# jeffreyhorn/network_flow_solver

Measured on AMD Instinct MI355X. Metric: pivots/sec + arcs-priced/sec (value = arcs-priced/sec; pivots_per_sec alongside) on netgen_8-style DIMACS, higher is better.
Workload: dtype int64; 1 GPU; netgen_8_08a(synthetic,x1): 256 nodes / 2048 arcs; pricing=full-scan Dantzig, step=one pivot (price + ratio test + tree/potential update), parallelism=1 GPU, sweeps=full (every arc priced every pivot)

## Files before the change

__graft_entry__.py:

```python

from __future__ import annotations

import os
import re
import subprocess
import sys
from pathlib import Path

ROOT = Path(__file__).resolve().parent
PKG = ROOT / "network_flow_solver_amd"
CSRC = PKG / "csrc"
LIB = PKG / "libmcf_hip.so"
CERT_HOST_LIB = PKG / "libmcf_certify_host.so"
REPAIR_HOST_LIB = PKG / "libmcf_repair_host.so"
FARKAS_HOST_LIB = PKG / "libmcf_farkas_host.so"
TOPOLOGY_HOST_LIB = PKG / "libmcf_topology_host.so"
RANGES_HOST_LIB = PKG / "libmcf_ranges_host.so"
FLOW_RANGES_HOST_LIB = PKG / "libmcf_flow_ranges_host.so"
DUAL_HOST_LIB = PKG / "libmcf_dual_host.so"
APPLY_PATHS_HOST_LIB = PKG / "libmcf_apply_paths_host.so"
SMALL_REDUCE_HOST_LIB = PKG / "libmcf_small_reduce_host.so"
SMALL_CYCLE_REGS_HOST_LIB = PKG / "libmcf_small_cycle_regs_host.so"
FORK_HOST_LIB = PKG / "libmcf_fork_host.so"
DECIDE_FLAT_HOST_LIB = PKG / "libmcf_decide_flat_host.so"
SMALL_SLOTS_HOST_LIB = PKG / "libmcf_small_slots_host.so"
SMALL_BUDGET_HOST_LIB = PKG / "libmcf_small_budget_host.so"

if str(ROOT) not in sys.path:
    sys.path.insert(0, str(ROOT))


def _hipcc() -> str:
    for cand in (os.environ.get("HIPCC"), "/opt/rocm/bin/hipcc", "hipcc"):
        if cand and (os.path.isabs(cand) and os.path.exists(cand) or not os.path.isabs(cand)):
            return cand
    return "hipcc"


def _needs_rebuild(target: Path, sources) -> bool:
    if not target.exists():
        return True
    t = target.stat().st_mtime
    return any(Path(s).stat().st_mtime > t for s in sources)


def build_hip(force: bool = False) -> Path:
    sources = [CSRC / "mcf_engine.hip", CSRC / "mcf_passes_dev.h", CSRC / "mcf_passes_host.h", CSRC / "mcf_core.h", CSRC / "mcf_host.h",
               ROOT / "include" / "mcf.h"]
    if force or _needs_rebuild(LIB, sources):
        cmd = [_hipcc(), "--offload-arch=gfx950", "-O3", "-std=c++17", "-fPIC", "-shared",
               "-o", str(LIB), str(CSRC / "mcf_engine.hip")]
        subprocess.run(cmd, check=True, cwd=str(CSRC))
    return LIB


def build_certify_host(force: bool = False) -> Path:
    src = CSRC / "mcf_certify_host.cpp"
    if force or _needs_rebuild(CERT_HOST_LIB, [src, CSRC / "mcf_core.h"]):
        subprocess.run(["g++", "-O2", "-std=c++17", "-fPIC", "-shared", "-o", str(CERT_HOST_LIB), str(src)], check=True, cwd=str(CSRC))
    return CERT_HOST_LIB


def build_repair_host(force: bool = False) -> Path:
    src = CSRC / "mcf_repair_host.cpp"
    if force or _needs_rebuild(REPAIR_HOST_LIB, [src, CSRC / "mcf_core.h", CSRC / "mcf_host.h"]):
        subprocess.run(["g++", "-O2", "-std=c++17", "-fPIC", "-shared", "-o", str(REPAIR_HOST_LIB), str(src)], check=True, cwd=str(CSRC))
    return REPAIR_HOST_LIB


def build_farkas_host(force: bool = False) -> Path:
    src = CSRC / "mcf_farkas_host.cpp"
    if force or _needs_rebuild(FARKAS_HOST_LIB, [src, CSRC / "mcf_core.h"]):
        subprocess.run(["g++", "-O2", "-std=c++17", "-fPIC", "-shared", "-o", str(FARKAS_HOST_LIB), str(src)], check=True, cwd=str(CSRC))
    return FARKAS_HOST_LIB


def build_topology_host(force: bool = False) -> Path:
    src = CSRC / "mcf_topology_host.cpp"
    if force or _needs_rebuild(TOPOLOGY_HOST_LIB, [src, CSRC / "mcf_core.h", CSRC / "mcf_host.h"]):
# ... 19 lines not shown
    src = CSRC / "mcf_dual_host.cpp"
    if force or _needs_rebuild(DUAL_HOST_LIB, [src, CSRC / "mcf_core.h", CSRC / "mcf_host.h", ROOT / "include" / "mcf.h"]):
        subprocess.run(["g++", "-O2", "-std=c++17", "-fPIC", "-shared", "-o", str(DUAL_HOST_LIB), str(src)], check=True, cwd=str(CSRC))
    return DUAL_HOST_LIB


def build_apply_paths_host(force: bool = False) -> Path:
    src = CSRC / "mcf_apply_paths_host.cpp"
    if force or _needs_rebuild(APPLY_PATHS_HOST_LIB, [src, CSRC / "mcf_core.h", CSRC / "mcf_host.h"]):
        subprocess.run(["g++", "-O2", "-std=c++17", "-fPIC", "-shared", "-o", str(APPLY_PATHS_HOST_LIB), str(src)], check=True, cwd=str(CSRC))
    return APPLY_PATHS_HOST_LIB


def build_small_reduce_host(force: bool = False) -> Path:
    src = CSRC / "mcf_small_reduce_host.cpp"
    if force or _needs_rebuild(SMALL_REDUCE_HOST_LIB, [src, CSRC / "mcf_core.h"]):
        subprocess.run(["g++", "-O2", "-std=c++17", "-fPIC", "-shared", "-o", str(SMALL_REDUCE_HOST_LIB), str(src)], check=True, cwd=str(CSRC))
    return SMALL_REDUCE_HOST_LIB


def build_small_cycle_regs_host(force: bool = False) -> Path:
    src = CSRC / "mcf_small_cycle_regs_host.cpp"
    if force or _needs_rebuild(SMALL_CYCLE_REGS_HOST_LIB, [src, CSRC / "mcf_core.h"]):
        subprocess.run(["g++", "-O2", "-std=c++17", "-fPIC", "-shared", "-o", str(SMALL_CYCLE_REGS_HOST_LIB), str(src)], check=True, cwd=str(CSRC))
    return SMALL_CYCLE_REGS_HOST_LIB


def build_fork_host(force: bool = False) -> Path:
    src = CSRC / "mcf_fork_host.cpp"
    if force or _needs_rebuild(FORK_HOST_LIB, [src, CSRC / "mcf_core.h"]):
        subprocess.run(["g++", "-O2", "-std=c++17", "-fPIC", "-shared", "-o", str(FORK_HOST_LIB), str(src)], check=True, cwd=str(CSRC))
    return FORK_HOST_LIB


def build_decide_flat_host(force: bool = False) -> Path:
    src = CSRC / "mcf_decide_flat_host.cpp"
    if force or _needs_rebuild(DECIDE_FLAT_HOST_LIB, [src, CSRC / "mcf_core.h"]):
        subprocess.run(["g++", "-O2", "-std=c++17", "-fPIC", "-shared", "-o", str(DECIDE_FLAT_HOST_LIB), str(src)], check=True, cwd=str(CSRC))
    return DECIDE_FLAT_HOST_LIB


def build_small_slots_host(force: bool = False) -> Path:
    src = CSRC / "mcf_small_slots_host.cpp"
    if force or _needs_rebuild(SMALL_SLOTS_HOST_LIB, [src, CSRC / "mcf_core.h"]):
        subprocess.run(["g++", "-O2", "-std=c++17", "-fPIC", "-shared", "-o", str(SMALL_SLOTS_HOST_LIB), str(src)], check=True, cwd=str(CSRC))
    return SMALL_SLOTS_HOST_LIB


def build_small_budget_host(force: bool = False) -> Path:
    src = CSRC / "mcf_small_budget_host.cpp"
    if force or _needs_rebuild(SMALL_BUDGET_HOST_LIB, [src, CSRC / "mcf_core.h", CSRC / "mcf_host.h"]):
        subprocess.run(["g++", "-O2", "-std=c++17", "-fPIC", "-shared", "-o", str(SMALL_BUDGET_HOST_LIB), str(src)], check=True, cwd=str(CSRC))
    return SMALL_BUDGET_HOST_LIB


def declared_symbols() -> list[str]:
    text = (ROOT / "include" / "mcf.h").read_text()
    text = re.sub(r"/\*.*?\*/", "", text, flags=re.S)
    names = re.findall(r"\b(mcf_[a-z0-9_]+)\s*\(", text)
    return sorted(set(n for n in names if n != "mcf_progress_cb"))


def build() -> None:
    build_hip()
    import oracle

    oracle.build()
    oracle.build_emul()
    build_certify_host()
    build_repair_host()
    build_farkas_host()
    build_topology_host()
    build_ranges_host()
    build_flow_ranges_host()
    build_dual_host()
    build_apply_paths_host()
    build_small_reduce_host()
    build_small_cycle_regs_host()
    build_fork_host()
    build_decide_flat_host()
    build_small_slots_host()
    build_small_budget_host()
    import ctypes

    lib = ctypes.CDLL(str(LIB))
    missing = [s for s in declared_symbols() if not hasattr(lib, s)]
    if missing:
        raise RuntimeError(f"libmcf_hip.so lacks symbols declared in include/mcf.h: {missing}")
    import network_flow_solver_amd


def smoke() -> None:
    import numpy as np

    build_hip()
    import oracle
    from network_flow_solver_amd import engine, generators

    if engine.device_count() <= 0:
        raise RuntimeError("smoke() needs a GPU: no HIP device visible")
    inst = generators.netgen_style(256, 2048, seed=7)
    ref = oracle.solve_soa(inst, "dantzig")
    for rule in (engine.RULE_DANTZIG, engine.RULE_DEVEX_BLOCK, engine.RULE_CANDIDATE_LIST):
        with engine.McfEngine(inst.n, inst.tail, inst.head, inst.cost, inst.cap, inst.supply, rule=rule,
                              device=0) as eng:
            eng.solve()
            res = eng.result()
        assert res.status == ref["status"] == "optimal", (res.status, ref["status"])
        assert res.objective == int(round(ref["objective"])), (res.objective, ref["objective"])
        bal = inst.supply.astype(np.int64).copy()
        np.subtract.at(bal, inst.tail, res.flow)
        np.add.at(bal, inst.head, res.flow)
        assert not bal.any()
        rc = inst.cost + res.potential[inst.tail] - res.potential[inst.head]
        assert (rc[(res.flow > 0) & (res.flow < inst.cap)] == 0).all()
        assert (rc[(res.flow == 0) & (inst.cap > 0)] >= 0).all() and (rc[(res.flow == inst.cap) & (inst.cap > 0)] <= 0).all()
        print(f"smoke ok: rule={rule} objective={res.objective} pivots={res.stats['pivots']} "
              f"(oracle {ref['iterations']} pivots)")


if __name__ == "__main__":
    build()
    if len(sys.argv) > 1 and sys.argv[1] == "smoke":
        smoke()
```

network_flow_solver_amd/csrc/mcf_core.h:

```cpp
#pragma once
#include <stdint.h>

#if defined(__HIPCC__)
#define MCF_HD __host__ __device__ __forceinline__
#else
#define MCF_HD inline
#endif

#define MCF_INF ((int64_t)1 << 60)

#if defined(__HIP_DEVICE_COMPILE__)
#define mcf_double_bits(x) ((int64_t)__double_as_longlong(x))
#else
static inline int64_t mcf_double_bits(double x) { int64_t k; __builtin_memcpy(&k, &x, 8); return k; }
#endif

#if defined(__HIP_DEVICE_COMPILE__)
#define MCF_TEAM_BARRIER() __syncthreads()
#define MCF_ATOMIC_MIN64(p, x) atomicMin(reinterpret_cast<long long*>(p), (long long)(x))
#define MCF_ATOMIC_MIN32(p, x) atomicMin(reinterpret_cast<int*>(p), (int)(x))
#define MCF_ATOMIC_MAX32(p, x) atomicMax(reinterpret_cast<int*>(p), (int)(x))
#define MCF_ATOMIC_ADD32(p, x) atomicAdd(reinterpret_cast<int*>(p), (int)(x))
#define MCF_ATOMIC_MAX64(p, x) atomicMax(reinterpret_cast<long long*>(p), (long long)(x))
#define MCF_ATOMIC_OR32(p, x) atomicOr(reinterpret_cast<int*>(p), (int)(x))
// ... 1917 lines not shown
    }
}

MCF_HD void mcf_apply_catch_up_store_at(int32_t* dst, int32_t* pnext, int32_t j, int32_t nd) {
    dst[j] = nd;
    pnext[nd] = j;
}
MCF_HD void mcf_apply_catch_up_store(const McfView& v, const McfCtx& c, int32_t j, int32_t nd) {
    (c.cur ? v.order[0] : v.order[1])[j] = nd;
    (c.cur ? v.posbuf[0] : v.posbuf[1])[nd] = j;
}

MCF_HD void mcf_apply_one_paths_at(const McfView& v, const McfCtx& c, const McfNode* srec, const int32_t* spos, const int32_t* src,
                                   int32_t* dst, int32_t* pnext, int32_t j) {
    if (j >= c.lo && j < c.hi) {
        bool in_t2;
        int32_t dd;
        const int32_t i = mcf_apply_source_paths(c, srec, spos, j, &in_t2, &dd);
        const int32_t nd = src[i];
        dst[j] = nd;
        pnext[nd] = j;
        if (in_t2) {
            const int64_t pot = v.pi[nd];
            const int32_t dep = v.node[nd].depth;
            v.pi[nd] = pot + c.sigma;
            if (dd) v.node[nd].depth = dep + dd;
        }
    } else {
        mcf_apply_catch_up_store_at(dst, pnext, j, src[j]);
    }
}
MCF_HD void mcf_apply_one_paths(const McfView& v, const McfCtx& c, const McfNode* srec, const int32_t* spos, int32_t j) {
    const int32_t* src = c.cur ? v.order[1] : v.order[0];
    int32_t* dst = c.cur ? v.order[0] : v.order[1];
    int32_t* pnext = c.cur ? v.posbuf[0] : v.posbuf[1];
    if (j >= c.lo && j < c.hi) {
        bool in_t2;
        int32_t dd;
        const int32_t i = mcf_apply_source_paths(c, srec, spos, j, &in_t2, &dd);
        const int32_t nd = src[i];
        dst[j] = nd;
        pnext[nd] = j;
        if (in_t2) {
            const int64_t pot = v.pi[nd];
            const int32_t dep = v.node[nd].depth;
            v.pi[nd] = pot + c.sigma;
            if (dd) v.node[nd].depth = dep + dd;
        }
    } else {
        mcf_apply_catch_up_store(v, c, j, src[j]);
    }
}

MCF_HD void mcf_reach_reindex_block(const McfView& v, const int32_t* zs, int32_t b) {
    int32_t m = 0;
    for (int32_t j = b << MCF_REACH_SHIFT; j < ((b + 1) << MCF_REACH_SHIFT) && j < v.n_nodes; ++j) {
        const int32_t e = j + zs[j];
        if (e > m) m = e;
    }
    v.reach[b] = m;
}

typedef unsigned __int128 mcf_u128;

#define MCF_CERT_BOUNDS 1u
#define MCF_CERT_CONSERVATION 2u
#define MCF_CERT_DUAL 4u
#define MCF_CERT_OBJECTIVES 8u
#define MCF_CERT_BASIS 16u
#define MCF_CERT_PRICING 32u
#define MCF_CERT_ALL 63u
#define MCF_CERT_NONE INT64_MAX

struct McfCertArcAcc {
    int64_t neg_n, over_n, bnd_w, bnd_i;
    int64_t dlo_n, dlo_w, dlo_i;
    int64_t dup_n, dup_w, dup_i;
    int64_t basic_n, stf_n;
    int64_t rc_n, rc_bad, key_n, key_bad;
    int64_t sat_n;
    uint64_t primal_lo, primal_hi;
    uint64_t dcap_lo, dcap_hi;
};
struct McfCertNodeAcc {
    int64_t imb_n, imb_w, imb_i;
    int64_t art_basic, tree_rc_bad, shape_bad, strong_bad;
    uint64_t art_lo, art_hi;
    uint64_t dnode_lo, dnode_hi;
};
template <typename Acc>
constexpr int mcf_acc_words() {
    static_assert(sizeof(Acc) % 8 == 0, "accumulators are whole 8-byte words");
    return (int)(sizeof(Acc) / 8);
}

MCF_HD void mcf_cert_arc_init(McfCertArcAcc* a) {
    uint64_t* p = reinterpret_cast<uint64_t*>(a);
    for (int k = 0; k < mcf_acc_words<McfCertArcAcc>(); ++k) p[k] = 0;
    a->bnd_i = a->dlo_i = a->dup_i = MCF_CERT_NONE;
}
MCF_HD void mcf_cert_node_init(McfCertNodeAcc* a) {
    uint64_t* p = reinterpret_cast<uint64_t*>(a);
    for (int k = 0; k < mcf_acc_words<McfCertNodeAcc>(); ++k) p[k] = 0;
    a->imb_i = MCF_CERT_NONE;
}
MCF_HD void mcf_cert_worst(int64_t* w, int64_t* wi, int64_t mag, int64_t idx) {
// ... 338 lines not shown
```

network_flow_solver_amd/csrc/mcf_engine.hip:

```cpp
#include <hip/hip_runtime.h>

#include <algorithm>
#include <cerrno>
#include <cstddef>
#include <chrono>
#include <cstdio>
#include <cstdlib>
#include <cstring>
#include <mutex>
#include <new>
#include <string>
#include <vector>

#include "../../include/mcf.h"
#include "mcf_core.h"
#include "mcf_host.h"

namespace {

constexpr int kPriceThreads = 256;
constexpr int kPivotThreads = 1024;
constexpr int kReduceThreads = 256;
constexpr int kMidMaxNodes = 1536;
constexpr int kMidMaxArcsPerPivot = MCF_TUNER_MAX_ARCS + 1024;
// ... 1358 lines not shown
#define MCF_WAVE_T0() do {} while (0)
#define MCF_WAVE_STAMP(slot) do {} while (0)
#define MCF_WAVE_PROBE(word) do {} while (0)
#endif

struct alignas(8) SmallCycleAcc {
    int32_t c[16][2];
};
constexpr bool small_search_join(int threads) { return threads != 256; }

template <bool LAST>
__device__ __forceinline__ void small_ratio_side(const int64_t* res, int32_t n, int64_t* d_out, int32_t* k_out) {
    const int32_t lane = (int32_t)(threadIdx.x & 63);
    int64_t d = MCF_INF;
    int32_t k = -1;
    const int64_t r0 = lane < n ? res[lane] : MCF_INF;
    bool wide = !mcf_ratio_narrow_ok(r0);
    for (int32_t i = 64 + lane; i < n; i += 64) wide |= !mcf_ratio_narrow_ok(res[i]);
    if (__ballot(wide) == 0) {
        for (int32_t base = 0; base < n; base += 64) {
            const int32_t i = base + lane;
            const uint32_t key = mcf_ratio_key32(base == 0 ? r0 : (i < n ? res[i] : MCF_INF));
            const uint32_t mn = mcf_wave_min_u32(key);
            const uint64_t mask = __ballot(i < n && key == mn);
            mcf_ratio_take<LAST>(mcf_ratio_unkey32(mn), mask, base, d, k);
        }
        *d_out = d; *k_out = k;
        return;
    }
    for (int32_t base = 0; base < n; base += 64) {
        const int32_t i = base + lane;
        const int64_t r = i < n ? res[i] : INT64_MAX;
        const int64_t mn = -mcf_wave_max64(-r);
        const uint64_t mask = __ballot(r == mn);
        mcf_ratio_take<LAST>(mn, mask, base, d, k);
    }
    *d_out = d; *k_out = k;
}

constexpr bool small_search_one_branch(int threads) { return threads == 256; }

constexpr bool small_ratio_together(int threads) { return threads == 256 || threads == 1024; }
constexpr bool small_record_once(int threads) { return threads == 256; }
typedef int small_i32x4 __attribute__((ext_vector_type(4)));
constexpr bool small_ratio_one_trip(int threads) { return threads == 256; }
typedef int small_i32x2 __attribute__((ext_vector_type(2)));
#ifndef MCF_BUDGET_OFF
#define MCF_BUDGET_OFF 0
#endif
constexpr bool small_pair_arith(int threads, bool front) { return threads == 256 && front && !(MCF_BUDGET_OFF & 1); }
constexpr bool small_ballot_direct(int threads, bool front) { return threads == 256 && front && !(MCF_BUDGET_OFF & 2); }
constexpr bool small_counts_packed(int threads, bool front) { return threads == 256 && front && !(MCF_BUDGET_OFF & 4); }
constexpr bool small_finish_one_trip(int threads, bool front) { return small_pair_arith(threads, front) && !(MCF_BUDGET_OFF & 8); }

template <int THREADS, bool FRONT>
__device__ __forceinline__ void small_cycle_parallel(const McfView& v, SmallCycleAcc& A, int64_t* scratch, McfCycle& cy) {
    constexpr bool kScalar = small_scalar_control(THREADS);
    constexpr bool kSearchJoin = small_search_join(THREADS);
    constexpr bool kSearchOneBranch = small_search_one_branch(THREADS);
    constexpr bool kRatioTogether = small_ratio_together(THREADS);
    constexpr bool kRecordOnce = small_record_once(THREADS);
    constexpr bool kRatioOneTrip = kRatioTogether && small_ratio_one_trip(THREADS);
    constexpr bool kPairs = small_pair_arith(THREADS, FRONT) && kSearchOneBranch;
    constexpr bool kBallot = small_ballot_direct(THREADS, FRONT) && kSearchOneBranch && !kSearchJoin && kRatioOneTrip;
    constexpr bool kCounts = small_counts_packed(THREADS, FRONT) && kRatioOneTrip;
    const McfCtx* c = v.ctx;
    const int32_t d4 = mcf_pair_dist4(v.n_nodes), d16 = mcf_pair_dist16(v.n_nodes);
    const int32_t* pcur = kPairs ? v.posbuf[0] + mcf_pair_index(0, c->cur, d4) : (c->cur ? v.posbuf[1] : v.posbuf[0]);
    const int32_t du0 = cy.r0u.depth, dw0 = cy.r0w.depth;
    const int32_t pu = cy.p0u, pw = cy.p0w;
    const int32_t wave = (int32_t)threadIdx.x >> 6;
    const int32_t N = v.n_nodes;
    int64_t* const res1 = scratch;
    int64_t* const res2 = res1 + N;
    int32_t* const by_depth = reinterpret_cast<int32_t*>(res2 + N);
    int32_t n1w = 0, n2w = 0;
    const int32_t nx = kSearchJoin ? N : N - 1;
    const int32_t side4 = dw0 - du0 + d4, side16 = dw0 - du0 + d16;
    auto file_pairs = [&](bool au, const McfNode& rec, int32_t px, int32_t x) {
        const McfArcW a = v.arcw[rec.pred >> 1];
        const int32_t bit = mcf_pair_bit(!au), i0 = du0 - rec.depth;
        const int32_t i4 = mcf_pair_index(i0, bit, side4), i16 = mcf_pair_index(i0, bit, side16);
        v.path1[i4] = x; v.rec1[i16] = rec; v.ppos1[i4] = px;
        const bool loses = ((rec.pred & 1) != 0) == au;
        res1[i16] = loses ? a.flow : (a.cap >= MCF_INF ? MCF_INF : a.cap - a.flow);
    };
    for (int32_t x0 = 0; x0 < nx; x0 += THREADS) {
        const int32_t x = x0 + (int32_t)threadIdx.x;
        bool h1 = false, h2 = false;
        uint64_t b1 = 0, b2 = 0;
        if constexpr (kBallot) {
            const uint64_t bin = __builtin_amdgcn_ballot_w64(x < nx);
            const int32_t xi = min(x, nx - 1);
            const small_i32x4 raw = *reinterpret_cast<const small_i32x4*>(&v.node[xi]);
            McfNode rec;
            rec.parent = raw.x; rec.pred = raw.y; rec.size = raw.z; rec.depth = raw.w;
            const int32_t px = pcur[xi];
            const bool au = (uint32_t)(pu - px) < (uint32_t)rec.size, aw = (uint32_t)(pw - px) < (uint32_t)rec.size;
            const uint64_t bu = __builtin_amdgcn_ballot_w64(au) & bin, bw = __builtin_amdgcn_ballot_w64(aw) & bin;
            b1 = bu & ~bw; b2 = bw & ~bu;
            if (x < nx && au != aw) {
                if constexpr (kPairs) file_pairs(au, rec, px, x);
                else {
                    const McfArcW a = v.arcw[rec.pred >> 1];
                    const int32_t idx = (au ? du0 : dw0) - rec.depth;
                    (au ? v.path1 : v.path2)[idx] = x; (au ? v.rec1 : v.rec2)[idx] = rec; (au ? v.ppos1 : v.ppos2)[idx] = px;
                    const bool loses = ((rec.pred & 1) != 0) == au;
                    (au ? res1 : res2)[idx] = loses ? a.flow : (a.cap >= MCF_INF ? MCF_INF : a.cap - a.flow);
                }
            }
        } else if (x < nx) {
            McfNode rec;
            if (kRecordOnce) {
                const small_i32x4 raw = *reinterpret_cast<const small_i32x4*>(&v.node[x]);
                rec.parent = raw.x; rec.pred = raw.y; rec.size = raw.z; rec.depth = raw.w;
            } else rec = v.node[x];
            const int32_t px = pcur[x];
            const bool au = (uint32_t)(pu - px) < (uint32_t)rec.size, aw = (uint32_t)(pw - px) < (uint32_t)rec.size;
            if (au && aw) { if (kSearchJoin) by_depth[rec.depth] = x; }
            else if (kSearchOneBranch) {
                if constexpr (kPairs) {
// ... 376 lines not shown
        const uint64_t k = lane < kWaves ? mine.key : 0;
        b.key = (uint64_t)mcf_wave_max64((int64_t)k);
        const int32_t w = (int32_t)__builtin_ctzll((unsigned long long)__ballot(k == b.key));
        b.e = __builtin_amdgcn_readlane(mine.e, w);
        b.info = (uint32_t)__builtin_amdgcn_readlane((int32_t)mine.info, w);
    }
    key = (int64_t)(b.key >> 32);
    if (key > 0) {
        wx = small_record(b.info, key, (int32_t)~(uint32_t)b.key, b.e);
        arc = wx.arc;
    } else { key = 0; arc = -1; }
    key = uni64<kScalar>(key); arc = uni64<kScalar>(arc);
    wx.rc = uni64<kScalar>(wx.rc); wx.tail = uni32<kScalar>(wx.tail); wx.head = uni32<kScalar>(wx.head); wx.state = uni32<kScalar>(wx.state);
}

template <bool SCALAR> __device__ __forceinline__ void small_cycle_ends(McfCycle& cy) {
    cy.r0u = uni_node<SCALAR>(cy.r0u); cy.r0w = uni_node<SCALAR>(cy.r0w);
    cy.ru = cy.r0u; cy.rw = cy.r0w;
    cy.p0u = uni32<SCALAR>(cy.p0u); cy.p0w = uni32<SCALAR>(cy.p0w);
    cy.s0u = cy.p0u; cy.s0w = cy.p0w; cy.pu = cy.p0u; cy.pw = cy.p0w; cy.su = cy.p0u; cy.sw = cy.p0w;
}
constexpr bool small_catch_up_beside(int threads, bool front) { return threads == 256 && front; }
template <int THREADS, bool FRONT> __device__ __forceinline__ void small_apply(const McfView& v, const McfCtx& cx) {
    if (!cx.apply) return;
    constexpr bool kCatchUpBeside = small_catch_up_beside(THREADS, FRONT);
    const int32_t lo = cx.lo, hi = cx.hi, plo = cx.prev_lo, phi = cx.prev_hi;
    const int32_t jc = plo + (int32_t)threadIdx.x;
    const bool catch0 = kCatchUpBeside && jc < phi && (jc < lo || jc >= hi);
    int32_t ndc = 0;
    if constexpr (small_pair_arith(THREADS, FRONT)) {
        const int32_t d4 = mcf_pair_dist4(v.n_nodes), d16 = mcf_pair_dist16(v.n_nodes);
        const int32_t sbit = cx.pv_result - 1, nbit = cx.cur ^ 1;
        const McfNode* const srec = v.rec1 + mcf_pair_index(0, sbit, d16);
        const int32_t* const spos = v.ppos1 + mcf_pair_index(0, sbit, d4);
        const int32_t* const src = v.order[0] + mcf_pair_index(0, cx.cur, d4);
        int32_t* const dst = v.order[0] + mcf_pair_index(0, nbit, d4);
        int32_t* const pnext = v.posbuf[0] + mcf_pair_index(0, nbit, d4);
        if (catch0) ndc = src[jc];
        for (int32_t j = lo + threadIdx.x; j < hi; j += THREADS) mcf_apply_one_paths_at(v, cx, srec, spos, src, dst, pnext, j);
        if (catch0) mcf_apply_catch_up_store_at(dst, pnext, jc, ndc);
        for (int32_t j = jc + (kCatchUpBeside ? THREADS : 0); j < phi; j += THREADS)
            if (j < lo || j >= hi) mcf_apply_one_paths_at(v, cx, srec, spos, src, dst, pnext, j);
    } else {
        const McfNode* const srec = cx.pv_result == 1 ? v.rec1 : v.rec2;
        const int32_t* const spos = cx.pv_result == 1 ? v.ppos1 : v.ppos2;
        if (catch0) ndc = (cx.cur ? v.order[1] : v.order[0])[jc];
        for (int32_t j = lo + threadIdx.x; j < hi; j += THREADS) mcf_apply_one_paths(v, cx, srec, spos, j);
        if (catch0) mcf_apply_catch_up_store(v, cx, jc, ndc);
        for (int32_t j = jc + (kCatchUpBeside ? THREADS : 0); j < phi; j += THREADS)
            if (j < lo || j >= hi) mcf_apply_one_paths(v, cx, srec, spos, j);
    }
}

template <int THREADS> __device__ __forceinline__ void small_budget_check(const McfView& v, const McfView& g, McfCtx* c, int& s_any) {
    if (c->status == MCF_PIVOT_LIMIT && !c->limit_checked) {
        if (threadIdx.x == 0) s_any = 0;
        __syncthreads();
        int any = 0;
        for (int64_t i = threadIdx.x; i < g.m && !any; i += THREADS)
            if (v.state[i] && mcf_violation(v, i) > 0) any = 1;
        if (any) s_any = 1;
        __syncthreads();
        if (threadIdx.x == 0) { if (s_any) c->limit_checked = 1; else c->status = MCF_OPTIMAL; }
        __syncthreads();
    }
}

template <int THREADS, bool FRONT>
__device__ __forceinline__ void solve_small_body(const McfView& g, const SmallLayout& L, int32_t rule_in,
                                                 McfCand* __restrict__ list, int64_t cap, char* smem, McfCtx* host_ctx) {
    static_assert(THREADS == 256 || THREADS == 1024, "the two widths the loop is tuned and instantiated for");
    const int32_t rule = FRONT ? (int32_t)MCF_RULE_DANTZIG : rule_in;
#ifdef MCF_STAMPS
    unsigned long long stamps_[8] = {0, 0, 0, 0, 0, 0, 0, 0};
    unsigned long long last_ = __builtin_amdgcn_s_memtime();
    unsigned long long last_wave_ = 0;
    if (threadIdx.x == 0) { for (int i = 0; i < 24; ++i) mcf_stamp_acc[i] = 0; mcf_stamp_last = last_; }
#ifdef MCF_WAVE_STAMPS
    if (threadIdx.x < 16 * 6) (&mcf_wave_acc[0][0])[threadIdx.x] = 0;
#endif
#endif
    const SmallSizes sizes = small_sizes(g);
    McfView v = small_map_view<FRONT>(g, L, smem);
    small_copy_image<THREADS, true>(g, L, smem, v.weight != nullptr, sizes);
    __syncthreads();
    STAMP(0);

    McfCtx* const c = v.ctx;
    if (threadIdx.x == 0) arm_ctx(c, cap);
    __shared__ int32_t s_gran[MCF_NUM_BUCKETS][MCF_GRANULES + 1];
    const bool devex = !FRONT && rule == MCF_RULE_DEVEX_BLOCK && g.dx;
    small_load_granules<THREADS>(g, devex, s_gran);
    const bool listing = !FRONT && rule == MCF_RULE_CANDIDATE_LIST;
    __shared__ int64_t s_lk[MCF_NUM_BUCKETS], s_la[MCF_NUM_BUCKETS];
    if (listing && threadIdx.x < MCF_NUM_BUCKETS) { s_lk[threadIdx.x] = list[threadIdx.x].key; s_la[threadIdx.x] = list[threadIdx.x].arc; }
    __syncthreads();
    __shared__ int32_t s_gsum[MCF_GRANULES + 1];
    small_sum_granules(devex, s_gran, s_gsum);
    __syncthreads();
    constexpr bool kScalar = small_scalar_control(THREADS);
    const int64_t priced_all = uni32<kScalar>(s_gsum[MCF_GRANULES] - s_gsum[0]);

    constexpr int kPer = THREADS / MCF_NUM_BUCKETS;
    constexpr int kReg = small_reg_arcs(THREADS);
    static_assert(kPer == 32 || kPer % 64 == 0, "a head bucket's lanes are half a wave or whole waves");
    const int px = threadIdx.x / kPer, pl = threadIdx.x % kPer;
    const int sweep = FRONT ? (int)kSweepPlain
                            : (devex ? kSweepDevex : (rule != MCF_RULE_DEVEX_BLOCK && v.key_mode == MCF_KEY_PLAIN ? kSweepPlain : kSweepGeneric));
    int32_t r_tail[kReg], r_head[kReg], r_cost[kReg], r_orig[kReg];
    uint32_t r_info[kReg];
    int32_t r_n = 0;
    constexpr int kRegFew = small_reg_arcs_few(THREADS, FRONT);
    static_assert(kRegFew <= kReg, "the shorter unrolled sweep is a prefix of the longer");
    const bool even = FRONT && sweep == kSweepPlain && rule == MCF_RULE_DANTZIG;
    const int32_t r_step = even ? THREADS : kPer;
    const int32_t r_lo = even ? mcf_even_arc(s_gran[0][0], (int32_t)threadIdx.x, 0, THREADS) : s_gran[px][0] + pl;
    const int32_t r_hi = even ? s_gran[MCF_NUM_BUCKETS - 1][MCF_GRANULES] : s_gran[px][MCF_GRANULES];
    const bool r_few = even && uni32<kScalar>(mcf_even_reg_slots(s_gran[MCF_NUM_BUCKETS - 1][MCF_GRANULES] - s_gran[0][0], THREADS, kRegFew, kReg)) == kRegFew;
#pragma unroll
    for (int k = 0; k < kReg; ++k) {
        const int32_t i = r_lo + k * r_step;
        const bool on = sweep == kSweepPlain && i < r_hi;
        r_tail[k] = on ? v.tail[i] : 0; r_head[k] = on ? v.head[i] : 0; r_cost[k] = on ? v.cost[i] : 0; r_orig[k] = on ? v.orig[i] : 0;
        r_info[k] = small_info(r_tail[k], r_head[k], k);
        r_n += on ? 1 : 0;
    }
    typedef uint32_t small_u32x2 __attribute__((ext_vector_type(2)));
    small_u32x2 r_key[small_price_flat(THREADS, FRONT) ? kReg : 1];
    if constexpr (small_price_flat(THREADS, FRONT)) {
#pragma unroll
        for (int k = 0; k < kReg; ++k) { r_key[k].x = (uint32_t)~r_orig[k]; r_key[k].y = 0; }
    }
    const bool reg_plain = sweep == kSweepPlain;
    constexpr bool nar = FRONT;
    constexpr bool kDescOnce = small_desc_once(THREADS, FRONT);
    constexpr bool kDecideFlat = small_decide_flat(THREADS, FRONT);
    constexpr bool kPriceFlat = small_price_flat(THREADS, FRONT);
    constexpr bool kPairs = small_pair_arith(THREADS, FRONT);
    constexpr int kPriceChains = small_price_chains(THREADS, FRONT);
    constexpr bool hand = FRONT;
    const int32_t* const pi32 = reinterpret_cast<const int32_t*>(v.pi);
// ... 145 lines not shown
        }
        STAMP(2);
        MCF_SLOT_PROBE_HERE();
        if (cx.pivots < cx.max_pivots)
            cx.arcs_priced += minor ? (int64_t)MCF_NUM_BUCKETS : (devex ? (int64_t)uni32<kScalar>(s_gsum[bg1] - s_gsum[bg0]) : priced_all);
        MCF_PSTAMP(12);
        McfCycle cy;
        bool go;
        if constexpr (hand) go = mcf_pivot_begin_t<true>(v, key, arc, rule, &wx, &cy);
        else go = mcf_pivot_begin_t<true>(v, key, arc, rule, nullptr, &cy);
        small_ctx_uniform<kScalar>(cx);
        MCF_PSTAMP(13);
        if (!go) {
            STAMP(3);
            __syncthreads();
            STAMP(5);
            continue;
        }
        small_cycle_ends<kScalar>(cy);
        const int32_t deep = cy.r0u.depth > cy.r0w.depth ? cy.r0u.depth : cy.r0w.depth;
        if (v.n_nodes <= kSmallCycleMaxNodes && deep > 3) {
            small_cycle_parallel<THREADS, FRONT>(v, s_acc, scratch, cy);
            MCF_PSTAMP(15);
            if constexpr (kDecideFlat && kPairs) mcf_pivot_decide_flat_t<true>(v, mcf_view_paths(v), cy, mcf_pair_dist4(v.n_nodes), mcf_pair_dist16(v.n_nodes));
            else if constexpr (kDecideFlat) mcf_pivot_decide_flat(v, mcf_view_paths(v), cy);
            else mcf_pivot_decide(v, mcf_view_paths(v), cy);
        } else {
            if (threadIdx.x < 2) {
                const bool ok = pivot_climb_2lanes(v, &s_cy);
                if (threadIdx.x == 0) s_ok = ok ? 1 : 0;
            }
            __syncthreads();
            if (uni32<kScalar>(s_ok)) {
                cy = s_cy;
                uni_cycle<kScalar>(cy);
                mcf_pivot_decide(v, mcf_view_paths(v), cy);
            } else {
                cx.status = MCF_INTERNAL_ERROR;
            }
        }
        small_ctx_uniform<kScalar>(cx);
        if constexpr (!kDescOnce) { if (threadIdx.x == 0) small_desc_store(c, cx, adj2, adj3); }
        MCF_PSTAMP(16);
        STAMP(3);
        MCF_WAVE_STAMP(2);
        if ((int32_t)threadIdx.x >= THREADS - 64) {
            MCF_LAST_WAVE_BEGIN();
            if constexpr (kPairs) mcf_pivot_finish_pairs<small_finish_one_trip(THREADS, FRONT)>(v, mcf_view_paths(v), mcf_pair_dist4(v.n_nodes), mcf_pair_dist16(v.n_nodes), (int32_t)threadIdx.x - (THREADS - 64), 64);
            else mcf_pivot_finish_t<true>(v, mcf_view_paths(v), (int32_t)threadIdx.x - (THREADS - 64), 64);
            MCF_LAST_WAVE_STAMP();
            MCF_WAVE_STAMP(4);
        }
        STAMP(4);
        small_apply<THREADS, FRONT>(v, cx);
        MCF_WAVE_STAMP(3);
        __syncthreads();
        cx.apply = 0;
        STAMP(5);
    }
    if (threadIdx.x == 0) {
        small_ctx_store(c, cx);
        if constexpr (kDescOnce) small_desc_store_all(c, cx);
    }
    v.ctx = c;
    __syncthreads();
    __shared__ int s_any;
    small_budget_check<THREADS>(v, g, c, s_any);
    small_copy_image<THREADS, false>(g, L, smem, v.weight != nullptr, sizes);
    if (host_ctx) copy_words<THREADS>(host_ctx, smem + L.ctx, (uint32_t)sizeof(McfCtx));
    if (listing && threadIdx.x < MCF_NUM_BUCKETS) list[threadIdx.x] = McfCand{s_lk[threadIdx.x], s_la[threadIdx.x]};
#ifdef MCF_STAMPS
    STAMP(6);
    if (threadIdx.x == 0) {
        unsigned long long* out = reinterpret_cast<unsigned long long*>(g.rec1);
        for (int i = 0; i < 7; ++i) out[i] = stamps_[i];
        for (int i = 0; i < 24; ++i) g_pivot_stamps[i] += mcf_stamp_acc[i];
    }
    if (threadIdx.x == THREADS - 64) reinterpret_cast<unsigned long long*>(g.rec1)[7] = last_wave_;
#ifdef MCF_WAVE_STAMPS
    if (threadIdx.x < 16 * 6 && (int64_t)g.n_nodes * (int64_t)sizeof(McfNode) >= (8 + 16 * 6) * 8)
        reinterpret_cast<unsigned long long*>(g.rec1)[8 + threadIdx.x] = (&mcf_wave_acc[0][0])[threadIdx.x];
#endif
#endif
}

template <int THREADS, bool FRONT>
__global__ __launch_bounds__(THREADS) __attribute__((amdgpu_waves_per_eu(THREADS / 256, THREADS / 256))) void k_solve_small(McfView g, SmallLayout L, int32_t rule,
                                                          McfCand* __restrict__ list, int64_t cap, McfCtx* host_ctx) {
    extern __shared__ __attribute__((aligned(16))) char smem[];
    solve_small_body<THREADS, FRONT>(g, L, rule, list, cap, smem, host_ctx);
}

struct SmallJob {
    McfView g;
    SmallLayout L;
    int32_t rule;
    int32_t narrow;
    McfCand* list;
    int64_t cap;
    McfCtx* host_ctx;
};

template <int THREADS, bool FRONT>
__global__ __launch_bounds__(THREADS) __attribute__((amdgpu_waves_per_eu(THREADS / 256, THREADS / 256))) void k_solve_small_batch(const SmallJob* __restrict__ jobs) {
    extern __shared__ __attribute__((aligned(16))) char smem[];
    const SmallJob& J = jobs[blockIdx.x];
    solve_small_body<THREADS, FRONT>(J.g, J.L, J.rule, J.list, J.cap, smem, J.host_ctx);
}

__global__ void k_ctl(McfCtx* c, int64_t max_pivots, int resume) {
    c->max_pivots = max_pivots;
    c->limit_checked = 0;
    if (resume && c->status == MCF_PIVOT_LIMIT && c->pivots < max_pivots) c->status = MCF_RUNNING;
}

__global__ void k_copy16(const uint4* __restrict__ src, uint4* __restrict__ dst, int64_t n16) {
    const int64_t stride = (int64_t)gridDim.x * blockDim.x;
    for (int64_t i = (int64_t)blockIdx.x * blockDim.x + threadIdx.x; i < n16; i += stride) dst[i] = src[i];
}

// ... 2022 lines not shown
```

Before: 757.1 million arcs/s.

## Apply tree update per node via positions only, rebuild order at kernel exit

In the small single-block kernel, the per-pivot apply step now runs over nodes instead of preorder positions. Each thread computes its node's new position, potential and depth from the pivot's path pieces, which are broadcast across the wave with readlane, and writes only the position buffer. The double-buffered order/position arrays collapse to one position array, and the order arrays are rebuilt once at kernel exit. This drops per-pivot order scatter and buffer flipping, but every pivot now touches all nodes and may loop over k path pieces. A host twin checker and driver verify the new update against the existing path-based apply.

```diff
diff --git a/__graft_entry__.py b/__graft_entry__.py
--- a/__graft_entry__.py
+++ b/__graft_entry__.py
@@ -25,6 +25,7 @@
 DECIDE_FLAT_HOST_LIB = PKG / "libmcf_decide_flat_host.so"
 SMALL_SLOTS_HOST_LIB = PKG / "libmcf_small_slots_host.so"
 SMALL_BUDGET_HOST_LIB = PKG / "libmcf_small_budget_host.so"
+SMALL_TAIL_HOST_LIB = PKG / "libmcf_small_tail_host.so"
 
 if str(ROOT) not in sys.path:
     sys.path.insert(0, str(ROOT))
@@ -150,6 +151,13 @@
     if force or _needs_rebuild(SMALL_BUDGET_HOST_LIB, [src, CSRC / "mcf_core.h", CSRC / "mcf_host.h"]):
         subprocess.run(["g++", "-O2", "-std=c++17", "-fPIC", "-shared", "-o", str(SMALL_BUDGET_HOST_LIB), str(src)], check=True, cwd=str(CSRC))
     return SMALL_BUDGET_HOST_LIB
+
+
+def build_small_tail_host(force: bool = False) -> Path:
+    src = CSRC / "mcf_small_tail_host.cpp"
+    if force or _needs_rebuild(SMALL_TAIL_HOST_LIB, [src, CSRC / "mcf_core.h", CSRC / "mcf_host.h"]):
+        subprocess.run(["g++", "-O2", "-std=c++17", "-fPIC", "-shared", "-o", str(SMALL_TAIL_HOST_LIB), str(src)], check=True, cwd=str(CSRC))
+    return SMALL_TAIL_HOST_LIB
 
 
 def declared_symbols() -> list[str]:
@@ -179,6 +187,7 @@
     build_decide_flat_host()
     build_small_slots_host()
     build_small_budget_host()
+    build_small_tail_host()
     import ctypes
 
     lib = ctypes.CDLL(str(LIB))
diff --git a/network_flow_solver_amd/csrc/mcf_core.h b/network_flow_solver_amd/csrc/mcf_core.h
--- a/network_flow_solver_amd/csrc/mcf_core.h
+++ b/network_flow_solver_amd/csrc/mcf_core.h
@@ -1993,6 +1993,37 @@
     }
 }
 
+MCF_HD void mcf_apply_node_piece(int32_t b, int32_t vin_depth, int32_t i, int32_t pi_, int32_t zi, int32_t di, int32_t pp, int32_t zp,
+                                 int32_t p, bool* found, int32_t* newp, int32_t* ddepth) {
+    if (!*found && p >= pi_ && p < pi_ + zi) {
+        *found = true;
+        *ddepth = vin_depth + 1 + i - di;
+        *newp = b + (p - pi_) + ((i > 0 && p < pp) ? zp : 0);
+    }
+}
+MCF_HD int32_t mcf_apply_node_target(const McfCtx& c, const McfNode* srec, const int32_t* spos, int32_t p, bool* in_t2, int32_t* ddepth) {
+    const int32_t b = c.t2_new, S = c.t2_size, a0 = c.t2_old;
+    *in_t2 = false;
+    *ddepth = 0;
+    if (p < c.lo || p >= c.hi) return p;
+    if (p >= a0 && p < a0 + S) {
+        *in_t2 = true;
+        if (c.pv_k == 0) {
+            *ddepth = c.pv_dd0;
+            return b + (p - a0);
+        }
+        bool found = false;
+        int32_t newp = p, pp = 0, zp = 0;
+        for (int32_t i = 0; i <= c.pv_k; ++i) {
+            const int32_t pi_ = spos[i], zi = srec[i].size;
+            mcf_apply_node_piece(b, c.pv_vin_depth, i, pi_, zi, srec[i].depth, pp, zp, p, &found, &newp, ddepth);
+            pp = pi_; zp = zi;
+        }
+        return newp;
+    }
+    return b <= a0 ? p + S : p - S;
+}
+
 MCF_HD void mcf_reach_reindex_block(const McfView& v, const int32_t* zs, int32_t b) {
     int32_t m = 0;
     for (int32_t j = b << MCF_REACH_SHIFT; j < ((b + 1) << MCF_REACH_SHIFT) && j < v.n_nodes; ++j) {
diff --git a/network_flow_solver_amd/csrc/mcf_engine.hip b/network_flow_solver_amd/csrc/mcf_engine.hip
--- a/network_flow_solver_amd/csrc/mcf_engine.hip
+++ b/network_flow_solver_amd/csrc/mcf_engine.hip
@@ -1434,6 +1434,10 @@
 constexpr bool small_ballot_direct(int threads, bool front) { return threads == 256 && front && !(MCF_BUDGET_OFF & 2); }
 constexpr bool small_counts_packed(int threads, bool front) { return threads == 256 && front && !(MCF_BUDGET_OFF & 4); }
 constexpr bool small_finish_one_trip(int threads, bool front) { return small_pair_arith(threads, front) && !(MCF_BUDGET_OFF & 8); }
+#ifndef MCF_TAIL_OFF
+#define MCF_TAIL_OFF 0
+#endif
+constexpr bool small_apply_by_node(int threads, bool front) { return small_pair_arith(threads, front) && !(MCF_TAIL_OFF & 1); }
 
 template <int THREADS, bool FRONT>
 __device__ __forceinline__ void small_cycle_parallel(const McfView& v, SmallCycleAcc& A, int64_t* scratch, McfCycle& cy) {
@@ -1448,7 +1452,8 @@
     constexpr bool kCounts = small_counts_packed(THREADS, FRONT) && kRatioOneTrip;
     const McfCtx* c = v.ctx;
     const int32_t d4 = mcf_pair_dist4(v.n_nodes), d16 = mcf_pair_dist16(v.n_nodes);
-    const int32_t* pcur = kPairs ? v.posbuf[0] + mcf_pair_index(0, c->cur, d4) : (c->cur ? v.posbuf[1] : v.posbuf[0]);
+    const int32_t* pcur = small_apply_by_node(THREADS, FRONT) ? v.posbuf[0]
+                        : (kPairs ? v.posbuf[0] + mcf_pair_index(0, c->cur, d4) : (c->cur ? v.posbuf[1] : v.posbuf[0]));
     const int32_t du0 = cy.r0u.depth, dw0 = cy.r0w.depth;
     const int32_t pu = cy.p0u, pw = cy.p0w;
     const int32_t wave = (int32_t)threadIdx.x >> 6;
@@ -1931,6 +1936,50 @@
     }
 }
 
+template <int THREADS> __device__ __forceinline__ void small_apply_nodes(const McfView& v, const McfCtx& cx) {
+    if (!cx.apply) return;
+    const int32_t d4 = mcf_pair_dist4(v.n_nodes), d16 = mcf_pair_dist16(v.n_nodes);
+    const int32_t sbit = cx.pv_result - 1;
+    const McfNode* const srec = v.rec1 + mcf_pair_index(0, sbit, d16);
+    const int32_t* const spos = v.ppos1 + mcf_pair_index(0, sbit, d4);
+    int32_t* const pos = v.posbuf[0];
+    const int32_t lo = cx.lo, hi = cx.hi, a0 = cx.t2_old, b = cx.t2_new, S = cx.t2_size, k = cx.pv_k;
+    const int32_t slide = b <= a0 ? S : -S;
+    const int32_t lane = (int32_t)(threadIdx.x & 63);
+    const int32_t nx = v.n_nodes - 1;
+    for (int32_t x0 = 0; x0 < nx; x0 += THREADS) {
+        const int32_t x = x0 + (int32_t)threadIdx.x;
+        const int32_t xi = min(x, nx - 1);
+        const int32_t p = pos[xi];
+        const int64_t pot = v.pi[xi];
+        const int32_t dep = v.node[xi].depth;
+        const bool live = x < nx;
+        const bool moved = live && (uint32_t)(p - lo) < (uint32_t)(hi - lo);
+        const bool t2 = live && (uint32_t)(p - a0) < (uint32_t)S;
+        int32_t newp = t2 ? b + (p - a0) : p + slide;
+        int32_t dd = cx.pv_dd0;
+        if (k > 0 && __ballot(t2) != 0) {
+            bool found = !t2;
+            int32_t pp = 0, zp = 0;
+            for (int32_t base = 0; base <= k; base += 64) {
+                const int32_t il = min(base + lane, k);
+                const int32_t sp_l = spos[il], sz_l = srec[il].size, sd_l = srec[il].depth;
+                const int32_t cnt = min(64, k + 1 - base);
+                for (int32_t q = 0; q < cnt; ++q) {
+                    const int32_t pq = __builtin_amdgcn_readlane(sp_l, q), zq = __builtin_amdgcn_readlane(sz_l, q), dq = __builtin_amdgcn_readlane(sd_l, q);
+                    mcf_apply_node_piece(b, cx.pv_vin_depth, base + q, pq, zq, dq, pp, zp, p, &found, &newp, &dd);
+                    pp = pq; zp = zq;
+                }
+            }
+        }
+        if (moved) pos[x] = newp;
+        if (t2) {
+            v.pi[x] = pot + cx.sigma;
+            if (dd) v.node[x].depth = dep + dd;
+        }
+    }
+}
+
 template <int THREADS> __device__ __forceinline__ void small_budget_check(const McfView& v, const McfView& g, McfCtx* c, int& s_any) {
     if (c->status == MCF_PIVOT_LIMIT && !c->limit_checked) {
         if (threadIdx.x == 0) s_any = 0;
@@ -1961,11 +2010,16 @@
 #endif
     const SmallSizes sizes = small_sizes(g);
     McfView v = small_map_view<FRONT>(g, L, smem);
+    constexpr bool kByNode = small_apply_by_node(THREADS, FRONT);
+    if constexpr (kByNode) v.posbuf[1] = v.posbuf[0];
     small_copy_image<THREADS, true>(g, L, smem, v.weight != nullptr, sizes);
     __syncthreads();
     STAMP(0);
 
     McfCtx* const c = v.ctx;
+    if constexpr (kByNode) {
+        if (c->cur ^ (c->pending_flip ? 1 : 0)) copy_words<THREADS>(smem + L.pos0, smem + L.pos1, sizes.N * 4u);
+    }
     if (threadIdx.x == 0) arm_ctx(c, cap);
     __shared__ int32_t s_gran[MCF_NUM_BUCKETS][MCF_GRANULES + 1];
     const bool devex = !FRONT && rule == MCF_RULE_DEVEX_BLOCK && g.dx;
@@ -2217,7 +2271,8 @@
             MCF_WAVE_STAMP(4);
         }
         STAMP(4);
-        small_apply<THREADS, FRONT>(v, cx);
+        if constexpr (kByNode) small_apply_nodes<THREADS>(v, cx);
+        else small_apply<THREADS, FRONT>(v, cx);
         MCF_WAVE_STAMP(3);
         __syncthreads();
         cx.apply = 0;
@@ -2231,6 +2286,18 @@
     __syncthreads();
     __shared__ int s_any;
     small_budget_check<THREADS>(v, g, c, s_any);
+    if constexpr (kByNode) {
+        int32_t* const o0 = reinterpret_cast<int32_t*>(smem + L.order0);
+        int32_t* const o1 = reinterpret_cast<int32_t*>(smem + L.order1);
+        const int32_t* const p0 = reinterpret_cast<const int32_t*>(smem + L.pos0);
+        int32_t* const p1 = reinterpret_cast<int32_t*>(smem + L.pos1);
+        for (uint32_t x = threadIdx.x; x < sizes.N; x += THREADS) {
+            const int32_t p = p0[x];
+            p1[x] = p;
+            if ((uint32_t)p < sizes.N) { o0[p] = (int32_t)x; o1[p] = (int32_t)x; }
+        }
+        __syncthreads();
+    }
     small_copy_image<THREADS, false>(g, L, smem, v.weight != nullptr, sizes);
     if (host_ctx) copy_words<THREADS>(host_ctx, smem + L.ctx, (uint32_t)sizeof(McfCtx));
     if (listing && threadIdx.x < MCF_NUM_BUCKETS) list[threadIdx.x] = McfCand{s_lk[threadIdx.x], s_la[threadIdx.x]};
diff --git a/network_flow_solver_amd/csrc/mcf_small_tail_driver.cpp b/network_flow_solver_amd/csrc/mcf_small_tail_driver.cpp
--- /dev/null
+++ b/network_flow_solver_amd/csrc/mcf_small_tail_driver.cpp
@@ -0,0 +1,53 @@
+#include <cstdint>
+#include <cstdio>
+#include <vector>
+
+extern "C" int32_t mcf_tail_target_host(int32_t lo, int32_t hi, int32_t t2_old, int32_t t2_new, int32_t t2_size, int32_t pv_k, int32_t vin_depth,
+                                        int32_t dd0, const int32_t* spos, const int32_t* ssize, const int32_t* sdepth, int32_t p, int32_t* in_t2,
+                                        int32_t* ddepth);
+extern "C" int mcf_tail_twin_host(int32_t n, int64_t m, const int32_t* tail, const int32_t* head, const int64_t* cost, const int64_t* cap,
+                                  const int64_t* supply, int64_t max_pivots, int64_t* report);
+
+int main() {
+    int bad = 0;
+    {
+        const int32_t spos[3] = {17, 14, 10}, ssize[3] = {3, 10, 20}, sdepth[3] = {9, 8, 7};
+        const int32_t order[20] = {17, 18, 19, 14, 15, 16, 20, 21, 22, 23, 10, 11, 12, 13, 24, 25, 26, 27, 28, 29};
+        int32_t wrong = 0;
+        std::vector<int32_t> hit(32, 0);
+        for (int32_t p = 0; p < 32; ++p) {
+            int32_t t2 = 0, dd = 0;
+            const int32_t np = mcf_tail_target_host(3, 30, 10, 3, 20, 2, 4, 4 + 1 - 9, spos, ssize, sdepth, p, &t2, &dd);
+            int32_t want = p;
+            if (p >= 3 && p < 10) want = p + 20;
+            for (int32_t j = 0; j < 20; ++j) if (order[j] == p) want = 3 + j;
+            if (np != want || (t2 != 0) != (p >= 10 && p < 30) || np < 0 || np >= 32) wrong += 1;
+            else hit[(size_t)np] += 1;
+        }
+        for (int32_t h : hit) if (h != 1) wrong += 1;
+        if (wrong) bad = 1;
+        std::printf("planted: 32 positions, wrong %d\n", wrong);
+    }
+    const int32_t sizes[5] = {2, 47, 64, 256, 513};
+    for (uint32_t seed = 1; seed <= 5; ++seed) {
+        const int32_t n = sizes[seed - 1];
+        std::vector<int32_t> tail, head;
+        std::vector<int64_t> cost, cap, supply((size_t)n, 0);
+        uint32_t x = seed * 2654435761u;
+        auto rnd = [&](uint32_t mod) { x = x * 1664525u + 1013904223u; return (x >> 8) % mod; };
+        for (int32_t u = 0; u < n; ++u) {
+            tail.push_back(u); head.push_back((u + 1) % n); cost.push_back(1 + rnd(50)); cap.push_back(2 + rnd(6));
+            for (int c = 0; c < (n > 100 ? 1 : 3); ++c) {
+                tail.push_back(u); head.push_back((u + 1 + (int32_t)rnd((uint32_t)n - 1)) % n); cost.push_back(1 + rnd(90)); cap.push_back(1 + rnd(4));
+            }
+        }
+        for (int32_t u = 0; u + 1 < n; u += 2) { const int64_t s = 1 + rnd(3); supply[(size_t)u] += s; supply[(size_t)((u * 7 + 3) % n)] -= s; }
+        int64_t r[24];
+        const int rc = mcf_tail_twin_host(n, (int64_t)tail.size(), tail.data(), head.data(), cost.data(), cap.data(), supply.data(), -1, r);
+        if (rc != 0 || r[3] != 0 || r[4] != 0 || r[5] != 0 || r[0] == 0 || (r[1] > 0 && r[18] < 1)) bad = 1;
+        std::printf("twin %d nodes: rc %d pivots %lld swaps %lld flips %lld bad_ctx %lld bad_tree %lld bad_arrays %lld k0 %lld k1 %lld k2 %lld k8+ %lld left %lld right %lld max_range %lld status %lld\n",
+                    n + 1, rc, (long long)r[0], (long long)r[1], (long long)r[2], (long long)r[3], (long long)r[4], (long long)r[5], (long long)r[8],
+                    (long long)r[9], (long long)r[10], (long long)r[11], (long long)r[12], (long long)r[13], (long long)r[21], (long long)r[6]);
+    }
+    return bad;
+}
diff --git a/network_flow_solver_amd/csrc/mcf_small_tail_host.cpp b/network_flow_solver_amd/csrc/mcf_small_tail_host.cpp
--- /dev/null
+++ b/network_flow_solver_amd/csrc/mcf_small_tail_host.cpp
@@ -0,0 +1,211 @@
+#include <cstdint>
+#include <cstring>
+#include <string>
+#include <vector>
+
+#include "mcf_host.h"
+
+namespace {
+
+template <typename T> T* at(std::vector<unsigned char>& buf, uint32_t off) { return reinterpret_cast<T*>(buf.data() + off); }
+
+template <typename T>
+bool same(const std::vector<T>& a, const T* b) { return a.empty() || std::memcmp(a.data(), b, a.size() * sizeof(T)) == 0; }
+
+struct Twin {
+    McfHostImage im;
+    std::vector<int32_t> order1, pos1, path1, path2, ppos1, ppos2;
+    std::vector<McfNode> rec1, rec2;
+    std::vector<McfSeg> seg;
+    McfCtx ctx_a, ctx_b;
+    McfView a{}, b{};
+    McfSmallLayout L;
+    std::vector<unsigned char> buf;
+};
+
+void bind_common(McfView& v, const McfHostImage& im, McfCtx* ctx, int64_t max_pivots) {
+    v.n_nodes = im.n_nodes;
+    v.m = im.m;
+    v.tail = im.tail.data(); v.head = im.head.data(); v.cost = im.cost.data(); v.orig = im.orig.data();
+    for (int x = 0; x <= MCF_NUM_BUCKETS; ++x) v.bucket_off[x] = im.bucket_off[x];
+    v.key_mode = MCF_KEY_PLAIN;
+    v.vk_bigm = im.big_m; v.vk_half = 1 << 28;
+    std::memset(ctx, 0, sizeof *ctx);
+    ctx->unbounded_arc = -1;
+    ctx->max_pivots = max_pivots < 0 ? INT64_MAX : max_pivots;
+    mcf_init_block_state(ctx, MCF_RULE_DANTZIG, im.m, 0);
+    ctx->climb_budget = INT32_MAX;
+    ctx->climb_depth = 0;
+    v.ctx = ctx;
+}
+
+bool bind(Twin& t, int64_t max_pivots) {
+    McfHostImage& im = t.im;
+    const size_t N = (size_t)im.n_nodes;
+    if (!mcf_small_plan(im.m_pad, (uint64_t)im.arcw.size(), im.n_nodes, false, &t.L)) return false;
+    t.order1 = im.order; t.pos1 = im.pos;
+    t.path1.assign(N, 0); t.path2.assign(N, 0); t.ppos1.assign(N, 0); t.ppos2.assign(N, 0);
+    t.rec1.assign(N, McfNode{0, 0, 0, 0}); t.rec2.assign(N, McfNode{0, 0, 0, 0});
+    t.seg.assign(2 * N + 2, McfSeg{0, 0, 0, 0});
+    t.buf.assign(t.L.total, 0xa5);
+    const McfSmallLayout& L = t.L;
+    std::memcpy(at<int8_t>(t.buf, L.state), im.state.data(), im.state.size());
+    std::memcpy(at<McfArcW>(t.buf, L.arcw), im.arcw.data(), im.arcw.size() * sizeof(McfArcW));
+    std::memcpy(at<int64_t>(t.buf, L.pi), im.pi.data(), N * 8);
+    std::memcpy(at<McfNode>(t.buf, L.node), im.node.data(), N * 16);
+    std::memcpy(at<int32_t>(t.buf, L.pos0), im.pos.data(), N * 4);
+    bind_common(t.a, im, &t.ctx_a, max_pivots);
+    bind_common(t.b, im, &t.ctx_b, max_pivots);
+    McfView& a = t.a;
+    a.state = im.state.data(); a.arcw = im.arcw.data(); a.pi = im.pi.data(); a.node = im.node.data();
+    a.order[0] = im.order.data(); a.order[1] = t.order1.data(); a.posbuf[0] = im.pos.data(); a.posbuf[1] = t.pos1.data();
+    a.path1 = t.path1.data(); a.path2 = t.path2.data(); a.ppos1 = t.ppos1.data(); a.ppos2 = t.ppos2.data();
+    a.rec1 = t.rec1.data(); a.rec2 = t.rec2.data(); a.seg = t.seg.data();
+    McfView& b = t.b;
+    b.state = at<int8_t>(t.buf, L.state); b.arcw = at<McfArcW>(t.buf, L.arcw); b.pi = at<int64_t>(t.buf, L.pi); b.node = at<McfNode>(t.buf, L.node);
+    b.order[0] = nullptr; b.order[1] = nullptr;
+    b.posbuf[0] = at<int32_t>(t.buf, L.pos0); b.posbuf[1] = b.posbuf[0];
+    b.path1 = at<int32_t>(t.buf, L.path1); b.path2 = at<int32_t>(t.buf, L.path2);
+    b.ppos1 = at<int32_t>(t.buf, L.ppos1); b.ppos2 = at<int32_t>(t.buf, L.ppos2);
+    b.rec1 = at<McfNode>(t.buf, L.rec1); b.rec2 = at<McfNode>(t.buf, L.rec2); b.seg = at<McfSeg>(t.buf, L.seg);
+    return true;
+}
+
+void price(const McfView& v, int64_t* key, int64_t* arc, int64_t* priced) {
+    int64_t bk = 0, ba = -1, np = 0;
+    for (int x = 0; x < MCF_NUM_BUCKETS; ++x) {
+        int64_t lo, hi;
+        mcf_bucket_slice(v.bucket_off, x, 0, 1, 0, 1, &lo, &hi);
+        np += hi - lo;
+        for (int64_t i = lo; i < hi; ++i) {
+            if (!v.state[i]) continue;
+            const int64_t viol = mcf_violation(v, i);
+            if (viol <= 0) continue;
+            const int64_t id = mcf_pack_arc(v.orig[i], i);
+            if (mcf_cand_better(viol, id, bk, ba)) { bk = viol; ba = id; }
+        }
+    }
+    *key = bk; *arc = ba; *priced = np;
+}
+
+bool same_tree(const Twin& t, std::vector<int32_t>& rebuilt) {
+    const McfCtx& ca = t.ctx_a;
+    const int32_t sel = ca.cur ^ (ca.pending_flip ? 1 : 0);
+    const int32_t N = t.im.n_nodes;
+    const int32_t* pa = sel ? t.pos1.data() : t.im.pos.data();
+    const int32_t* oa = sel ? t.order1.data() : t.im.order.data();
+    const int32_t* pb = t.b.posbuf[0];
+    rebuilt.assign((size_t)N, -1);
+    for (int32_t x = 0; x < N; ++x) {
+        if (pa[x] != pb[x] || pb[x] < 0 || pb[x] >= N) return false;
+        rebuilt[(size_t)pb[x]] = x;
+    }
+    return std::memcmp(rebuilt.data(), oa, (size_t)N * 4) == 0;
+}
+
+bool same_arrays(const Twin& t) {
+    const McfHostImage& im = t.im;
+    const McfView& b = t.b;
+    return same(im.state, b.state) && same(im.arcw, b.arcw) && same(im.pi, b.pi) && same(im.node, b.node);
+}
+
+}
+
+extern "C" {
+
+int32_t mcf_tail_target_host(int32_t lo, int32_t hi, int32_t t2_old, int32_t t2_new, int32_t t2_size, int32_t pv_k, int32_t vin_depth,
+                             int32_t dd0, const int32_t* spos, const int32_t* ssize, const int32_t* sdepth, int32_t p, int32_t* in_t2, int32_t* ddepth) {
+    McfCtx c;
+    std::memset(&c, 0, sizeof c);
+    c.lo = lo; c.hi = hi; c.t2_old = t2_old; c.t2_new = t2_new; c.t2_size = t2_size; c.pv_k = pv_k; c.pv_vin_depth = vin_depth; c.pv_dd0 = dd0;
+    std::vector<McfNode> srec((size_t)pv_k + 1, McfNode{0, 0, 0, 0});
+    for (int32_t i = 0; i <= pv_k; ++i) { srec[(size_t)i].size = ssize[i]; srec[(size_t)i].depth = sdepth[i]; }
+    bool t2 = false;
+    const int32_t np = mcf_apply_node_target(c, srec.data(), spos, p, &t2, ddepth);
+    *in_t2 = t2 ? 1 : 0;
+    return np;
+}
+
+int mcf_tail_twin_host(int32_t n, int64_t m, const int32_t* tail, const int32_t* head, const int64_t* cost, const int64_t* cap,
+                       const int64_t* supply, int64_t max_pivots, int64_t* report) {
+    if (!report) return -1;
+    for (int k = 0; k < 24; ++k) report[k] = 0;
+    report[7] = -1;
+    report[18] = INT32_MAX;
+    Twin t;
+    int code = 0;
+    if (!mcf_build_image(n, m, tail, head, cost, cap, supply, t.im, &code).empty()) return -1;
+    if (!bind(t, max_pivots)) return 1;
+    const int32_t N = t.im.n_nodes;
+    report[23] = N;
+    const int32_t d4 = mcf_pair_dist4(N), d16 = mcf_pair_dist16(N);
+    McfCtx &ca = t.ctx_a, &cb = t.ctx_b;
+    std::vector<int32_t> rebuilt;
+    auto flag = [&](int which) { report[which] += 1; if (report[7] < 0) report[7] = ca.pivots; };
+    while (ca.status == MCF_RUNNING) {
+        int64_t key, arc, priced, keyb, arcb, pricedb;
+        price(t.a, &key, &arc, &priced);
+        price(t.b, &keyb, &arcb, &pricedb);
+        if (key != keyb || arc != arcb) { flag(5); break; }
+        if (ca.pivots < ca.max_pivots) { ca.arcs_priced += priced; cb.arcs_priced += priced; }
+        mcf_pivot_walk(t.a, key, arc, MCF_RULE_DANTZIG);
+        if (mcf_pivot_begin(t.b, key, arc, MCF_RULE_DANTZIG)) {
+            McfCycle cy;
+            mcf_cycle_init(t.b, &cy);
+            if (!mcf_pivot_climb(t.b, mcf_view_paths(t.b), &cy, mcf_climb_budget(t.b, cy)) || cy.u != cy.w) return -2;
+            mcf_pivot_decide_flat_t<true>(t.b, mcf_view_paths(t.b), cy, d4, d16);
+        }
+        if (std::memcmp(&ca, &cb, sizeof(McfCtx)) != 0) { flag(3); break; }
+        if (ca.status == MCF_INTERNAL_ERROR) return -2;
+        if (ca.stage == 2) {
+            report[1] += 1;
+            if (ca.pv_k <= 2) report[8 + ca.pv_k] += 1;
+            if (ca.pv_k >= 8) report[11] += 1;
+            report[ca.t2_new <= ca.t2_old ? 12 : 13] += 1;
+            if (ca.t2_size == 1) report[14] += 1;
+            if (ca.t2_size > 64) report[15] += 1;
+            if (ca.lo == 1) report[16] += 1;
+            if (ca.hi == N) report[17] += 1;
+            if (ca.lo < report[18]) report[18] = ca.lo;
+            if (ca.pv_k > report[20]) report[20] = ca.pv_k;
+            if (ca.hi - ca.lo > report[21]) report[21] = ca.hi - ca.lo;
+            if (ca.cur) report[22] += 1;
+        } else if (ca.stage == 1) {
+            report[2] += 1;
+        }
+        mcf_pivot_finish_t<true>(t.a, mcf_view_paths(t.a), 0, 1);
+        for (int32_t lane = 0; lane < 64; ++lane) mcf_pivot_finish_pairs<true>(t.b, mcf_view_paths(t.b), d4, d16, lane, 64);
+        if (ca.apply) {
+            const McfNode* sa = ca.pv_result == 1 ? t.a.rec1 : t.a.rec2;
+            const int32_t* pa = ca.pv_result == 1 ? t.a.ppos1 : t.a.ppos2;
+            for (int32_t j = ca.lo; j < ca.hi; ++j) mcf_apply_one_paths(t.a, ca, sa, pa, j);
+            for (int32_t j = ca.prev_lo; j < ca.prev_hi; ++j)
+                if (j < ca.lo || j >= ca.hi) mcf_apply_one_paths(t.a, ca, sa, pa, j);
+            const int32_t sbit = cb.pv_result - 1;
+            const McfNode* sb = t.b.rec1 + mcf_pair_index(0, sbit, d16);
+            const int32_t* pb = t.b.ppos1 + mcf_pair_index(0, sbit, d4);
+            int32_t* pos = t.b.posbuf[0];
+            for (int32_t x = 0; x < N - 1; ++x) {
+                bool in_t2;
+                int32_t dd;
+                const int32_t p = pos[x];
+                const int32_t np = mcf_apply_node_target(cb, sb, pb, p, &in_t2, &dd);
+                report[19] += 1;
+                if (np != p) pos[x] = np;
+                if (in_t2) {
+                    t.b.pi[x] += cb.sigma;
+                    if (dd) t.b.node[x].depth += dd;
+                }
+            }
+        }
+        if (std::memcmp(&ca, &cb, sizeof(McfCtx)) != 0) flag(3);
+        if (!same_tree(t, rebuilt)) flag(4);
+        if (!same_arrays(t)) flag(5);
+    }
+    if (report[18] == INT32_MAX) report[18] = -1;
+    report[0] = ca.pivots;
+    report[6] = ca.status;
+    return 0;
+}
+
+}
```

New measurement: 697.0 million arcs/s. -7.9%, worse.
